# sunyzhi55/Diffusion_Models_Collection

Hardware: AMD Instinct MI355X
Metric: CIFAR-10 UNet DDPM train imgs/sec (aggregate over GPUs) (higher is better)
Workload: dtype bf16; 1 GPU; configs/cifar10_unet.py UNet DDPM train step at 32x32 (q_sample, fwd, MSE, bwd, clip, AdamW, EMA), dropout 0.1; model=UNet 37.06M (128ch, mult 1,2,2,2, attn 16/8), global_batch=128, per_gpu_batch=128, parallelism=dp1

## Files before the change

diffusion_models_collection_amd/_lib.py:

```python
import ctypes
import os
from pathlib import Path

import torch

_PKG = Path(__file__).resolve().parent
LIB_PATH = Path(os.environ.get("DMC_LIB", _PKG / "libdmc.so"))

DMC_F32, DMC_BF16 = 0, 1
MODE_NORMAL, MODE_UPSAMPLE, MODE_DILATE = 0, 1, 2
PRO_NONE, PRO_AFFINE_SILU, PRO_SILU, PRO_AFFINE, PRO_GN_SILU = 0, 1, 2, 3, 4
LOSS = {"l1": 0, "l2": 1, "huber": 2}
PRED = {"eps": 0, "v": 1}
OBJECTIVE_MAX_BLOCKS = 64
PACK_FWD, PACK_DGRAD, PACK_UPDGRAD = 0, 1, 2

_c_int, _c_p, _c_f, _c_u32, _c_long, _c_size = (ctypes.c_int, ctypes.c_void_p, ctypes.c_float, ctypes.c_uint32,
                                                ctypes.c_long, ctypes.c_size_t)


ACT_NONE, ACT_GELU, ACT_GELU_DROP, ACT_DGELU = 0, 1, 2, 3
FUSED_GN_STATS = 1


class ConvDesc(ctypes.Structure):
    _fields_ = [
        ("dtype", _c_int), ("N", _c_int), ("H", _c_int), ("W", _c_int),
        ("C1", _c_int), ("C2", _c_int), ("ld1", _c_int), ("ld2", _c_int), ("Kc", _c_int),
        ("OH", _c_int), ("OW", _c_int), ("Cout", _c_int), ("ntaps", _c_int), ("mode", _c_int), ("stride", _c_int),
        ("tap_dy", _c_int * 16), ("tap_dx", _c_int * 16),
        ("prologue", _c_int), ("pro_scale", _c_p), ("pro_shift", _c_p), ("ld_pro", _c_int),
        ("drop_seed", _c_u32), ("drop_thresh", _c_u32), ("drop_scale", _c_f), ("drop_ld", _c_int),
        ("drop_seed_base", _c_p),
        ("bias", _c_p), ("addvec", _c_p), ("ld_add", _c_int), ("resid", _c_p), ("ld_res", _c_int),
        ("silu_pre", _c_p), ("ld_silu", _c_int), ("Csplit", _c_int), ("ldy1", _c_int), ("ldy2", _c_int),
        ("out_f32", _c_int), ("out_nchw", _c_int), ("act", _c_int), ("y_pre", _c_p), ("ld_pre", _c_int),
        ("gn_part", _c_p), ("wg_bias", _c_p), ("pro_groups", _c_int), ("pro_eps", _c_f),
    ]


class WgradJob(ctypes.Structure):
    _fields_ = [("slab", ctypes.c_void_p), ("bslab", ctypes.c_void_p), ("dw", ctypes.c_void_p),
                ("dbias", ctypes.c_void_p), ("splits", ctypes.c_int), ("KK", ctypes.c_int), ("Cpad", ctypes.c_int),
                ("Cout", ctypes.c_int), ("Ctot", ctypes.c_int), ("ntaps", ctypes.c_int), ("Kc", ctypes.c_int),
                ("scale", ctypes.c_float), ("layout", ctypes.c_int)]
# ... 18 lines not shown
    _fields_ = [("w", _c_p), ("dst", _c_p), ("dtype", _c_int), ("mode", _c_int), ("Cout", _c_int), ("Cin", _c_int),
                ("kh", _c_int), ("kw", _c_int), ("Kc", _c_int), ("koff", _c_int)]


class TensorRef(ctypes.Structure):
    _fields_ = [("a", _c_p), ("b", _c_p), ("n", _c_long)]


def _load():
    if not LIB_PATH.exists():
        raise RuntimeError(
            f"libdmc.so not found at {LIB_PATH}. Build it with `python -m diffusion_models_collection_amd.build` "
            "(there is no fallback: the diffusion hot path runs only on the gfx950 HIP kernels).")
    lib = ctypes.CDLL(str(LIB_PATH))
    sig = {
        "dmc_version": (_c_int, []),
        "dmc_set_option": (_c_int, [ctypes.c_char_p, _c_long]),
        "dmc_get_option": (_c_long, [ctypes.c_char_p]),
        "dmc_reset_options": (None, [_c_int]),
        "dmc_last_error": (ctypes.c_char_p, []),
        "dmc_conv2d_workspace": (_c_size, [ctypes.POINTER(ConvDesc)]),
        "dmc_conv_halo_prologue": (_c_int, [ctypes.POINTER(ConvDesc)]),
        "dmc_conv2d_fused_epilogue": (_c_int, [ctypes.POINTER(ConvDesc), ctypes.c_size_t]),
        "dmc_conv2d": (_c_int, [ctypes.POINTER(ConvDesc), _c_p, _c_p, _c_p, _c_p, _c_p, _c_p, _c_size, _c_p]),
        "dmc_conv2d_wgrad_workspace": (_c_size, [ctypes.POINTER(ConvDesc)]),
        "dmc_conv2d_wgrad": (_c_int, [ctypes.POINTER(ConvDesc), _c_p, _c_int, _c_p, _c_p, _c_p, _c_p, _c_f, _c_p]),
        "dmc_conv2d_wgrad_partial": (_c_int, [ctypes.POINTER(ConvDesc), _c_p, _c_int, _c_p, _c_p, _c_p, _c_p, _c_f,
                                              ctypes.POINTER(WgradJob), _c_p]),
        "dmc_wgrad_reduce_batch": (_c_int, [ctypes.POINTER(WgradJob), _c_int, _c_p]),
        "dmc_conv2d_wgrad_group_ok": (_c_int, [ctypes.POINTER(ConvDesc), _c_int]),
        "dmc_conv2d_wgrad_group_workspace": (_c_size, [ctypes.POINTER(WgradGroupItem), _c_int,
                                                       ctypes.POINTER(_c_size)]),
        "dmc_conv2d_wgrad_group": (_c_int, [ctypes.POINTER(WgradGroupItem), _c_int, ctypes.POINTER(WgradJob), _c_p]),
        "dmc_wgrad_slab_bytes": (_c_long, [_c_int]),
        "dmc_pack_weight": (_c_int, [_c_int, _c_int, _c_p, _c_int, _c_int, _c_int, _c_int, _c_int, _c_p, _c_p]),
        "dmc_pack_tiles": (_c_int, [ctypes.POINTER(PackJob), _c_int, _c_p, _c_int]),
        "dmc_pack_weights": (_c_int, [_c_p, _c_p, _c_int, _c_p]),
        "dmc_gn_workspace": (_c_size, [_c_int, _c_int, _c_int, _c_int]),
        "dmc_gn_stats": (_c_int, [_c_int, _c_p, _c_p, _c_int, _c_int, _c_int, _c_int, _c_int, _c_int, _c_int, _c_f,
                                  _c_p, _c_p, _c_p, _c_p, _c_p, _c_p, _c_p]),
        "dmc_gn_finalize": (_c_int, [_c_p, _c_int, _c_p, _c_int, _c_int, _c_int, _c_int, _c_f, _c_p, _c_p, _c_p, _c_p,
                                     _c_p, _c_p]),
        "dmc_gn_stats_apply_ok": (_c_int, [_c_int, _c_int, _c_int, _c_int, _c_int, _c_int]),
        "dmc_gn_stats_apply": (_c_int, [_c_int, _c_p, _c_p, _c_int, _c_int, _c_int, _c_int, _c_int, _c_int, _c_int,
                                        _c_f, _c_p, _c_p, _c_p, _c_p, _c_p, _c_int, _c_u32, _c_p, _c_u32, _c_f, _c_p,
                                        _c_int, _c_p]),
# ... 143 lines not shown
```

diffusion_models_collection_amd/csrc/dmc_conv.hip:

```cpp
#include "dmc_conv_impl.h"

namespace {

template <typename T> DMC_DEV void load4(const char* p, size_t idx, float* v, bool f32);
template <typename T>
DMC_DEV void load4(const char* p, size_t idx, float* v, bool f32) {
  if (f32 || sizeof(T) == 4) {
    v4f x = *(const v4f*)(p + idx * 4);
    v[0] = x[0]; v[1] = x[1]; v[2] = x[2]; v[3] = x[3];
  } else {
    v2i x = *(const v2i*)(p + idx * 2);
    v[0] = bf2f((uint32_t)x[0] & 0xffffu); v[1] = bf2f((uint32_t)x[0] >> 16);
    v[2] = bf2f((uint32_t)x[1] & 0xffffu); v[3] = bf2f((uint32_t)x[1] >> 16);
  }
}
template <typename T>
DMC_DEV void store4(char* p, size_t idx, const float* v, bool f32) {
  if (f32 || sizeof(T) == 4) {
    v4f x = {v[0], v[1], v[2], v[3]};
    *(v4f*)(p + idx * 4) = x;
  } else {
    v2i x;
    x[0] = (int)f2bf2(v[0], v[1]);
    x[1] = (int)f2bf2(v[2], v[3]);
// ... 428 lines not shown
template <int AI, int BI, int BM>
DMC_DEV void glds_issue_buf(const ConvK& a, char* base, int c0, unsigned k2, int wave, const unsigned* o1,
                            const unsigned* o2, const unsigned* ob) {
  if (c0 < a.C1) {
    const __amdgpu_buffer_rsrc_t r = __builtin_amdgcn_make_buffer_rsrc((void*)a.x1, (short)0, a.x1_bytes, 0x00020000);
    const unsigned c2 = (unsigned)c0 * 2u;
#pragma unroll
    for (int j = 0; j < AI; ++j)
      __builtin_amdgcn_raw_ptr_buffer_load_lds(r, (LDS_AS void*)(base + (wave * AI + j) * 1024), 16, o1[j] + c2, 0, 0, 0);
  } else {
    const __amdgpu_buffer_rsrc_t r = __builtin_amdgcn_make_buffer_rsrc((void*)a.x2, (short)0, a.x2_bytes, 0x00020000);
    const unsigned c2 = (unsigned)(c0 - a.C1) * 2u;
#pragma unroll
    for (int j = 0; j < AI; ++j)
      __builtin_amdgcn_raw_ptr_buffer_load_lds(r, (LDS_AS void*)(base + (wave * AI + j) * 1024), 16, o2[j] + c2, 0, 0, 0);
  }
  const __amdgpu_buffer_rsrc_t rw = __builtin_amdgcn_make_buffer_rsrc((void*)a.w, (short)0, a.w_bytes, 0x00020000);
#pragma unroll
  for (int j = 0; j < BI; ++j)
    __builtin_amdgcn_raw_ptr_buffer_load_lds(rw, (LDS_AS void*)(base + BM * 128 + (wave * BI + j) * 1024), 16, ob[j] + k2, 0, 0, 0);
}

DMC_DEV void xcd_tile(int NB, int& mb, int& nb) {
  const int total = gridDim.x, bid = blockIdx.x, per = total >> 3;
  const int t = bid < (per << 3) ? (bid & 7) * per + (bid >> 3) : bid;
  mb = t / NB;
  nb = t - mb * NB;
}

__host__ __device__ inline bool reg_epi_ok(const ConvK& a) {
  return a.reg_epi && (a.gst || a.reg_epi >= 2) && a.dtype_bytes == 2 && !a.out_f32 && !a.out_nchw && !a.silu_pre && a.Csplit == a.Cout &&
         a.act == DMC_ACT_NONE && (a.Cout & 127) == 0 && (a.ldy1 & 7) == 0 &&
         (!a.resid || (a.ld_res & 7) == 0) && (a.M & 127) == 0 && (!a.gst || a.OHW % 64 == 0);
}
DMC_DEV void reg_epilogue(const ConvK& a, v4f (&acc)[4][4], int m0, int n0, int wm, int wn) {
  const int lane = threadIdx.x & 63, fr = lane & 15, fh = lane >> 4;
  const bool odd = fh & 1;
  v4i rra[4][2];
  v4f ba[4], eva[4];
  const int img0 = (m0 + wm * 64) / a.OHW;
#pragma unroll
  for (int i = 0; i < 4; ++i) {
    const int co = n0 + wn * 64 + i * 16 + fh * 4;
    const int cc = co - (odd ? 4 : 0);
#pragma unroll
    for (int jp = 0; jp < 2; ++jp) {
      rra[i][jp] = v4i{0, 0, 0, 0};
      if (a.resid) {
// ... 211 lines not shown
      reg_epilogue(a, acc, m0, n0, wm, wn);
      return;
    }
  }
  __syncthreads();
#pragma unroll
  for (int j = 0; j < 4; ++j)
#pragma unroll
    for (int i = 0; i < 4; ++i)
      *(v4f*)(lds + (wm * 64 + j * 16 + fr) * EP + (wn * 64 + i * 16 + fh * 4) * 4) = acc[i][j];
  __syncthreads();
  if (a.sk) {
    const int Cpad = gridDim.y * BN;
    float* slab = a.sk + (size_t)blockIdx.z * a.M * Cpad;
    for (int idx = threadIdx.x; idx < BM * BN / 4; idx += NW * 64) {
      const int pl = idx / (BN / 4), cg = idx - pl * (BN / 4);
      if (m0 + pl < a.M) *(v4f*)(slab + (size_t)(m0 + pl) * Cpad + n0 + cg * 4) = *(const v4f*)(lds + pl * EP + cg * 16);
    }
    return;
  }
  tile_epilogue<T, BM, BN, NW * 64>(a, lds, EP, m0, n0);
}

DMC_DEV void wait_vm_upto40(int n) {
  switch (n < 0 ? 0 : n) {
#define DMC_W(i) case i: __builtin_amdgcn_s_waitcnt(waitcnt_vm(i)); break;
    DMC_W(0) DMC_W(1) DMC_W(2) DMC_W(3) DMC_W(4) DMC_W(5) DMC_W(6) DMC_W(7) DMC_W(8) DMC_W(9) DMC_W(10)
    DMC_W(11) DMC_W(12) DMC_W(13) DMC_W(14) DMC_W(15) DMC_W(16) DMC_W(17) DMC_W(18) DMC_W(19) DMC_W(20)
    DMC_W(21) DMC_W(22) DMC_W(23) DMC_W(24) DMC_W(25) DMC_W(26) DMC_W(27) DMC_W(28) DMC_W(29) DMC_W(30)
    DMC_W(31) DMC_W(32) DMC_W(33) DMC_W(34) DMC_W(35) DMC_W(36) DMC_W(37) DMC_W(38) DMC_W(39)
#undef DMC_W
    default: __builtin_amdgcn_s_waitcnt(waitcnt_vm(40)); break;
  }
}

template <int NS>
__global__ __launch_bounds__(256, NS <= 2 ? 2 : 1) void gemm1x1_persist_kernel(ConvK a, int ntiles, int NB, int tpb) {
  using T = bf16_t;
  constexpr int BM = 128, BN = 128, AI = 4, BI = 4, SB = (BM + BN) * 128;
  __shared__ __attribute__((aligned(16))) char lds[NS * SB + 4096];
  float* const sbias = (float*)(lds + NS * SB);
  const int lane = threadIdx.x & 63;
  const int wave = __builtin_amdgcn_readfirstlane(threadIdx.x >> 6);
  const int wm = wave % 2, wn = wave / 2;
  const int lrow = lane >> 3, lc = (lane & 7) ^ lrow;
  const int fr = lane & 15, fh = lane >> 4;
  const int t_begin = blockIdx.x * tpb, t_end = min(ntiles, t_begin + tpb);
  if (t_begin >= t_end) return;
  const int kst = a.Kc / 64, total = (t_end - t_begin) * kst;
  for (int c = threadIdx.x; c < NB * BN; c += 256) sbias[c] = (a.bias && c < a.Cout) ? a.bias[c] : 0.f;
  __builtin_amdgcn_s_waitcnt(waitcnt_vm(0));

  unsigned o1[AI], o2[AI], ob[BI];
  int it_tile = -1;
  auto issue = [&](int S) {
    const int ti = t_begin + S / kst, k = S - (S / kst) * kst;
    if (ti != it_tile) {
      it_tile = ti;
      const int mb = ti / NB, nb = ti - mb * NB;
#pragma unroll
      for (int j = 0; j < AI; ++j) {
        const unsigned pix = (unsigned)(mb * BM + (wave * AI + j) * 8 + lrow);
        o1[j] = (pix * a.ld1 + lc * 8) * 2u;
        o2[j] = (pix * a.ld2 + lc * 8) * 2u;
      }
#pragma unroll
      for (int j = 0; j < BI; ++j) {
        const unsigned co = (unsigned)(nb * BN + (wave * BI + j) * 8 + lrow);
        ob[j] = (co * a.Kc + lc * 8) * 2u;
      }
    }
    glds_issue_buf<AI, BI, BM>(a, lds + (S % NS) * SB, k * 64, (unsigned)k * 128u, wave, o1, o2, ob);
  };
  int nvm = 0;
  int pos[NS];
#pragma unroll
  for (int q = 0; q < NS; ++q) pos[q] = 0;
  for (int q = 0; q < NS - 1 && q < total; ++q) {
    issue(q);
    nvm += AI + BI;
    pos[q] = nvm;
  }
  v4f acc[4][4];
#pragma unroll
  for (int i = 0; i < 4; ++i)
#pragma unroll
    for (int j = 0; j < 4; ++j) acc[i][j] = v4f{0.f, 0.f, 0.f, 0.f};
  for (int s = 0; s < total; ++s) {
    int mine = 0;
#pragma unroll
    for (int q = 0; q < NS; ++q)
      if (q == s % NS) mine = pos[q];
    wait_vm_upto40(nvm - mine);
    asm volatile("" ::: "memory");
    __builtin_amdgcn_sched_barrier(0);
    __builtin_amdgcn_s_barrier();
    __builtin_amdgcn_sched_barrier(0);
    asm volatile("" ::: "memory");
    v2i rres[4][4];
    const bool last = (s + 1) % kst == 0;
    if (a.resid && last) {
      const int t = t_begin + s / kst, mb = t / NB, nb = t - mb * NB;
#pragma unroll
      for (int i = 0; i < 4; ++i)
#pragma unroll
        for (int j = 0; j < 4; ++j) {
          const int co = nb * BN + wn * 64 + i * 16 + fh * 4, px = mb * BM + wm * 64 + j * 16 + fr;
          rres[i][j] = *(const v2i*)(a.resid + ((size_t)px * a.ld_res + co) * 2);
        }
      nvm += 16;
      asm volatile("" ::: "memory");
    }
    if (s + NS - 1 < total) {
      issue(s + NS - 1);
      nvm += AI + BI;
#pragma unroll
// ... 42 lines not shown
      for (int i = 0; i < 4; ++i) {
        const int co = n0 + wn * 64 + i * 16 + fh * 4;
        const v4f bv = *(const v4f*)(sbias + co);
#pragma unroll
        for (int j = 0; j < 4; ++j) {
          const int px = m0 + wm * 64 + j * 16 + fr;
          v4f v = acc[i][j] + bv;
          if (a.resid) {
            const v2i r = rres[i][j];
            v[0] += bf2f((uint32_t)r[0] & 0xffffu); v[1] += bf2f((uint32_t)r[0] >> 16);
            v[2] += bf2f((uint32_t)r[1] & 0xffffu); v[3] += bf2f((uint32_t)r[1] >> 16);
          }
          v2i o;
          o[0] = (int)f2bf2(v[0], v[1]);
          o[1] = (int)f2bf2(v[2], v[3]);
          *(v2i*)(ybase + ((size_t)px * ldy + co - cbase) * 2) = o;
          acc[i][j] = v4f{0.f, 0.f, 0.f, 0.f};
        }
      }
      nvm += 16;
      asm volatile("" ::: "memory");
      __builtin_amdgcn_sched_barrier(0);
    }
  }
}



template <int HP>
DMC_DEV void halo_issue(const ConvK& a, char* buf, int c0, int wave, int pb, int pe, const unsigned* h1,
                        const unsigned* h2) {
  const bool first = c0 < a.C1;
  const __amdgpu_buffer_rsrc_t r = __builtin_amdgcn_make_buffer_rsrc(
      first ? (void*)a.x1 : (void*)a.x2, (short)0, first ? a.x1_bytes : a.x2_bytes, 0x00020000);
  const unsigned c2 = (unsigned)(first ? c0 : c0 - a.C1) * 2u;
#pragma unroll
  for (int p = 0; p < HP; ++p)
    if (p >= pb && p < pe)
      __builtin_amdgcn_raw_ptr_buffer_load_lds(r, (LDS_AS void*)(buf + (wave * HP + p) * 1024), 16,
                                               (first ? h1[p] : h2[p]) + c2, 0, 0, 0);
}

DMC_DEV void halo_pro_load(const ConvK& a, int n, int c0, v4f* st) {
  const int lane = threadIdx.x & 63, lrow = lane >> 3, lc = (lane & 7) ^ lrow;
  const float* sc = a.psc + (size_t)n * a.ldp + c0 + lc * 8;
  const float* sh = a.psh + (size_t)n * a.ldp + c0 + lc * 8;
// ... 1153 lines not shown

bool epi_stats_ok(const ConvK& k, const void* ws, size_t ws_bytes) {
  if (k.dtype_bytes != 2 || k.out_f32 || k.out_nchw || k.silu_pre || k.Csplit != k.Cout || k.Cout % 128 ||
      k.M % 256 || k.OHW % 64 || ((k.Cout | k.ldy1 | k.ld_res) & 7))
    return false;
  if (!dmc::opt(dmc::OPT_NO_NARROW) && ((k.C2 == 0 && k.C1 <= 8 && k.Cout >= 16) || k.Cout <= 8)) {
    int R, nimg;
    return nin_plan(k, &R, &nimg) != 0;
  }
  if (dmc::opt(dmc::OPT_NO_GLDS) || dmc::opt(dmc::OPT_NO_EPI_STATS))
    return false;
  if (img_plan(k))
    return k.OH == 8 && k.act == DMC_ACT_NONE;
  if (k.prologue == DMC_PRO_AFFINE_SILU) {
    int R, nimg;
    return halo2_pro_plan(k, &R, &nimg) != 0;
  }
  if (k.prologue != DMC_PRO_NONE) return false;
  const FwdPlan p = plan_glds(k);
  return p.splits == 1 || ws == nullptr || ws_bytes < p.ws || dmc::opt(dmc::OPT_NO_SPLITK);
}


int gemm1x1_plan(const ConvK& k) {
  if (!dmc::opt(dmc::OPT_GEMM1X1) || k.dtype_bytes != 2 || k.ntaps != 1 || k.stride != 1 || k.mode != DMC_MODE_NORMAL ||
      k.tdy0 || k.tdx0 || k.H != k.OH || k.W != k.OW || k.prologue != DMC_PRO_NONE)
    return 0;
  if (k.C1 % 64 || k.C2 % 64 || k.Kc != k.C1 + k.C2 || k.x1_bytes == 0 || (k.C2 && k.x2_bytes == 0) || k.w_bytes == 0)
    return 0;
  if (k.addvec || (k.resid && (k.ld_res & 3)) || k.silu_pre || k.gst || k.gsk ||
      k.act != DMC_ACT_NONE || k.sk || k.out_f32 || k.out_nchw || (k.ldy1 & 3) || k.M % 128 ||
      k.Cout % 128 || k.Cout > 1024)
    return 0;
  if (k.Csplit != k.Cout && (k.Csplit % 128 || (k.ldy2 & 3) || !k.y2 || k.resid)) return 0;
  const long ntiles = (long)(k.M / 128) * (k.Cout / 128);
  if (ntiles < 128) return 0;
  const long blocks = 512;
  return (int)((ntiles + blocks - 1) / blocks);
}

template <typename T>
int launch_fwd(ConvK k, void* ws, size_t ws_bytes, hipStream_t s) {
  constexpr int EPC = TT<T>::KPL;
  DMC_REQUIRE(k.prologue != DMC_PRO_GN_SILU || img_plan(k),
              "conv: DMC_PRO_GN_SILU is taken only by the small-map conv (dmc_conv_halo_prologue says when)");
  if (!dmc::opt(dmc::OPT_NO_NARROW) && sizeof(T) == 2) {
    int R, nimg;
    if (k.C2 == 0 && k.C1 <= EPC && k.Cout >= 16 && nin_plan(k, &R, &nimg)) {
      if (reg_epi_ok(k)) conv3x3_nin_kernel<true><<<dim3(k.M / 128, k.Cout / 128), 256, 0, s>>>(k, R, nimg);
      else conv3x3_nin_kernel<false><<<dim3(k.M / 128, k.Cout / 128), 256, 0, s>>>(k, R, nimg);
      return dmc::check_launch("dmc_conv2d");
    }
    const int hp = k.Cout <= 8 ? nout_plan(k, &R, &nimg) : 0;
    if (hp) {
      const int npl = (k.C1 + k.C2) / 64;
      const dim3 g(k.M / 128);
      if (hp == 6) { if (npl == 1) conv3x3_nout_kernel<6, 1><<<g, 256, 0, s>>>(k, R, nimg); else conv3x3_nout_kernel<6, 2><<<g, 256, 0, s>>>(k, R, nimg); }
      else if (hp == 7) { if (npl == 1) conv3x3_nout_kernel<7, 1><<<g, 256, 0, s>>>(k, R, nimg); else conv3x3_nout_kernel<7, 2><<<g, 256, 0, s>>>(k, R, nimg); }
      else { if (npl == 1) conv3x3_nout_kernel<9, 1><<<g, 256, 0, s>>>(k, R, nimg); else conv3x3_nout_kernel<9, 2><<<g, 256, 0, s>>>(k, R, nimg); }
      return dmc::check_launch("dmc_conv2d");
    }
  }
  if (!dmc::opt(dmc::OPT_NO_NARROW)) {
    if (k.C2 == 0 && k.C1 <= EPC && k.Cout >= 16) {
      conv_narrow_in_kernel<T><<<dim3(dmc::cdiv(k.M, 256), dmc::cdiv(k.Cout, 32)), 256, 0, s>>>(k);
      return dmc::check_launch("dmc_conv2d");
    }
    if (k.Cout <= 8 && (k.C2 == 0 || k.C1 % EPC == 0)) {
      conv_narrow_out_kernel<T><<<dmc::cdiv(k.M, 256), 256, 0, s>>>(k);
      return dmc::check_launch("dmc_conv2d");
    }
  }
  if (sizeof(T) == 2) {
    const int bn = img_plan(k);
    if (bn) { launch_img(k, bn, s); return dmc::check_launch("dmc_conv2d"); }
  }
  if (sizeof(T) == 2) {
    const int tpb = gemm1x1_plan(k);
    if (tpb) {
      const int NB = k.Cout / 128, ntiles = (k.M / 128) * NB;
      gemm1x1_persist_kernel<2><<<dmc::cdiv(ntiles, tpb), 256, 0, s>>>(k, ntiles, NB, tpb);
      return dmc::check_launch("dmc_conv2d");
    }
  }
  if (sizeof(T) == 2 && k.prologue == DMC_PRO_AFFINE_SILU) {
    int R, nimg;
    const int hp2 = halo2_pro_plan(k, &R, &nimg);
    if (hp2) { launch_halo2<true>(k, hp2, R, nimg, s); return dmc::check_launch("dmc_conv2d"); }
  }
  if (sizeof(T) == 2 && k.prologue == DMC_PRO_NONE && !dmc::opt(dmc::OPT_NO_GLDS)) {
    FwdPlan p = plan_glds(k);
    if (p.splits > 1 && (ws == nullptr || ws_bytes < p.ws || dmc::opt(dmc::OPT_NO_SPLITK))) { p.splits = 1; p.cfg = 2; }
    if (p.splits > 1) { k.sk = (float*)ws; k.sk_per = p.per; }
    const bool buf = k.C1 % 64 == 0 && k.C2 % 64 == 0 && k.Kc == k.C1 + k.C2 && k.x1_bytes > 0 &&
                     (k.C2 == 0 || k.x2_bytes > 0) && k.w_bytes > 0 && !dmc::opt(dmc::OPT_NO_BUFLDS);
    int R2, nimg2;
    const int hp2 = (buf && p.splits == 1 && !dmc::opt(dmc::OPT_NO_HALO)) ? halo2_plan(k, &R2, &nimg2) : 0;
    if (hp2) launch_halo2<false>(k, hp2, R2, nimg2, s);
    else if (buf) launch_glds<true>(k, p, s);
    else launch_glds<false>(k, p, s);
    return dmc::check_launch("dmc_conv2d");
  }
  const RegPlan rp = plan_reg(k);
  if (rp.big) {
// ... 15 lines not shown
  return dmc::check_launch("dmc_conv2d");
}


}

extern "C" size_t dmc_conv2d_workspace(const dmc_conv_desc* d) {
  ConvK k;
  if (fill_convk(d, nullptr, nullptr, nullptr, nullptr, nullptr, k)) return 0;
  if (k.M == 0) return 0;
  if (d->dtype != DMC_BF16 || d->prologue != DMC_PRO_NONE || dmc::opt(dmc::OPT_NO_GLDS)) return plan_reg(k).ws;
  return plan_glds(k).ws;
}

extern "C" int dmc_conv2d_fused_epilogue(const dmc_conv_desc* d, size_t ws_bytes) {
  ConvK k;
  if (fill_convk(d, nullptr, nullptr, nullptr, nullptr, nullptr, k) || k.M == 0 || k.Cout == 0) return 0;
  const void* ws = ws_bytes ? (const void*)d : nullptr;
  int f = 0;
  if (k.OHW % 64 == 0 && k.Cout % 8 == 0 && epi_stats_ok(k, ws, ws_bytes)) f |= DMC_FUSED_GN_STATS;
  return f;
}

extern "C" int dmc_conv2d(const dmc_conv_desc* d, const void* x1, const void* x2, const void* w, void* y1,
                          void* y2, void* workspace, size_t ws_bytes, void* stream) {
  ConvK k;
  if (fill_convk(d, x1, x2, w, y1, y2, k)) return 1;
  hipStream_t s = dmc::as_stream(stream);
  if (k.M == 0 || k.Cout == 0) return 0;
  float* const part = d->gn_part;
  if (part) {
    DMC_REQUIRE(k.OHW % 64 == 0 && k.Cout % 8 == 0 && k.Csplit == k.Cout && !k.out_nchw && k.ldy1 % 4 == 0,
                "conv: GroupNorm partials need OH*OW %% 64 == 0, Cout %% 8 == 0 and one NHWC output");
    k.gst = epi_stats_ok(k, workspace, ws_bytes) ? part : nullptr;
  }
  int gsk_done = 0;
  if (part && !k.gst && !dmc::opt(dmc::OPT_NO_SKGN)) { k.gsk = part; k.gsk_done = &gsk_done; }
  const int rc = d->dtype == DMC_F32 ? launch_fwd<float>(k, workspace, ws_bytes, s)
                                     : launch_fwd<bf16_t>(k, workspace, ws_bytes, s);
  if (rc) return rc;
  if (!part || k.gst || gsk_done) return 0;
  const int nseg = k.M / 64, nch = k.Cout / 8;
  const int blocks = (int)(((long)nseg * nch + 3) / 4);
  if (k.out_f32 || d->dtype == DMC_F32)
    gn_part_kernel<float><<<blocks, 256, 0, s>>>(k.y1, k.ldy1, nseg, nch, part);
  else
// ... 53 lines not shown
```

diffusion_models_collection_amd/csrc/dmc_elem.hip:

```cpp
#include <stdlib.h>
#include <string.h>
#include "dmc_common.h"
#include "dmc_internal.h"

namespace dmc {
static thread_local char g_err[512] = "";
void set_error(const char* fmt, ...) {
  va_list ap;
  va_start(ap, fmt);
  vsnprintf(g_err, sizeof(g_err), fmt, ap);
  va_end(ap);
}
}

namespace dmc {
namespace {
struct OptDef {
  const char* name;
  long def;
};
constexpr OptDef kOpts[OPT_COUNT] = {
    {"DMC_NO_NARROW", 0}, {"DMC_NO_GLDS", 0}, {"DMC_NO_SPLITK", 0}, {"DMC_NO_BUFLDS", 0}, {"DMC_NO_HALO", 0},
    {"DMC_HALO_PRO", 1}, {"DMC_GN_STATS_SPLIT", 0}, {"DMC_GN_BWD_SPLIT", 0}, {"DMC_ATTN_STAGED", 0},
    {"DMC_ATTN_HG", 0}, {"DMC_WG_BLOCKS", 512}, {"DMC_GN_STATS_ONE_MAX", 1l << 20}, {"DMC_GN_BWD_ONE_MAX", 65536},
    {"DMC_NO_XCD", 0}, {"DMC_NO_EPI_STATS", 0}, {"DMC_WG_MINPIX", 0}, {"DMC_GN_BWD_SLICES", 2}, {"DMC_NO_SKGN", 0},
    {"DMC_WG_HALO_TARGET", 256}, {"DMC_SK_TARGET", 240}, {"DMC_SK_MAX", 8}, {"DMC_NO_NHALO", 0},
    {"DMC_GN_BWD_FUSED", 4}, {"DMC_GN_BWD_FUSED_MAXHW", 1l << 30}, {"DMC_GN_BWD_NT", 1024},
    {"DMC_REG_EPI", 3}, {"DMC_GEMM1X1", 1}, {"DMC_WG_PIPE", 1}, {"DMC_IMG_MASK", 15}, {"DMC_IMG_GN", 1}, {"DMC_WG_IMG4", 1},
};
struct OptTable {
  long v[OPT_COUNT];
  OptTable() { reset(true); }
  void reset(bool env) {
    for (int i = 0; i < OPT_COUNT; ++i) {
      v[i] = kOpts[i].def;
      const char* e = env ? getenv(kOpts[i].name) : nullptr;
      if (e && e[0]) v[i] = atol(e);
    }
  }
};
OptTable& table() {
  static OptTable t;
  return t;
}
}
long opt(Opt o) { return table().v[o]; }
}

extern "C" int dmc_set_option(const char* name, long value) {
  for (int i = 0; i < dmc::OPT_COUNT; ++i)
    if (strcmp(name, dmc::kOpts[i].name) == 0) {
// ... 897 lines not shown
```

diffusion_models_collection_amd/kernels.py:

```python
import ctypes

import torch

from . import _lib as L
from ._lib import LIB, check, ptr

TAPS3 = [(kh - 1, kw - 1) for kh in range(3) for kw in range(3)]
TAPS3_DGRAD = [(1 - kh, 1 - kw) for kh in range(3) for kw in range(3)]
TAPS1 = [(0, 0)]
TAPS_UPDGRAD = [(u - 1, v - 1) for u in range(4) for v in range(4)]


class Scratch:

    def __init__(self):
        self.bufs = {}

    def get(self, nbytes: int, device) -> torch.Tensor:
        nbytes = max(int(nbytes), 256)
        key = L.stream()
        buf = self.bufs.get(key)
        if buf is None or buf.numel() < nbytes:
            buf = torch.empty(int(nbytes * 1.25) + 4096, dtype=torch.uint8, device=device)
            self.bufs[key] = buf
# ... 84 lines not shown
        self.pending = []
        rows = sorted(agg.items(), key=lambda kv: -kv[1][1])
        tot = sum(v[1] for v in agg.values())
        lines = [f"conv launches: {tot / steps:.3f} ms/step"]
        for (kind, dt, N, H, W, Cin, OH, OW, Cout, nt, mode), (n, ms, fl) in rows:
            lines.append(f"{ms / steps * 1e3:8.1f} us/step  n/step {n / steps:4.1f}  avg {ms / n * 1e3:7.1f} us  "
                         f"{fl / (ms * 1e-3) / 1e12:7.1f} TF/s  {kind:5s} N{N} {H}x{W}x{Cin} -> {OH}x{OW}x{Cout} "
                         f"taps {nt} mode {mode}")
        return "\n".join(lines)


PROF = LayerProfile()


def conv(d, x1, x2, w, y1, y2=None):
    nbytes = LIB.dmc_conv2d_workspace(ctypes.byref(d))
    ws = SCRATCH.get(nbytes, y1.device) if nbytes else None
    PROF.wrap("conv", d, lambda: check(LIB.dmc_conv2d(ctypes.byref(d), ptr(x1), ptr(x2), ptr(w), ptr(y1), ptr(y2),
                                                      ptr(ws), nbytes, L.stream()), "dmc_conv2d"))


def conv_fused(d):
    return LIB.dmc_conv2d_fused_epilogue(ctypes.byref(d), LIB.dmc_conv2d_workspace(ctypes.byref(d)))


def upsample2x(dtype, x, C):
    N, H, W, ld = x.shape
    y = torch.empty(N, 2 * H, 2 * W, C, dtype=x.dtype, device=x.device)
    check(LIB.dmc_upsample2x_nhwc(L.dtype_code(dtype), ptr(x), N, H, W, C, ld, ptr(y), C, L.stream()),
          "dmc_upsample2x_nhwc")
    return y


def conv_halo_prologue(d):
    return bool(LIB.dmc_conv_halo_prologue(ctypes.byref(d)))


def _byte_span(t):
    n = 1 + sum((sz - 1) * st for sz, st in zip(t.shape, t.stride())) if t.numel() else 0
    return t.data_ptr(), t.data_ptr() + n * t.element_size()


class WgradDefer:

    def __init__(self):
        import os
# ... 720 lines not shown
```

include/dmc.h:

```cpp
#ifndef DMC_H
#define DMC_H
#include <stddef.h>
#include <stdint.h>
#ifdef __cplusplus
extern "C" {
#endif

enum { DMC_F32 = 0, DMC_BF16 = 1 };
enum { DMC_MODE_NORMAL = 0, DMC_MODE_UPSAMPLE = 1, DMC_MODE_DILATE = 2 };
enum { DMC_PRO_NONE = 0, DMC_PRO_AFFINE_SILU = 1, DMC_PRO_SILU = 2, DMC_PRO_AFFINE = 3, DMC_PRO_GN_SILU = 4 };
enum { DMC_LOSS_L1 = 0, DMC_LOSS_L2 = 1, DMC_LOSS_HUBER = 2 };
enum { DMC_PRED_EPS = 0, DMC_PRED_V = 1 };
#define DMC_OBJECTIVE_MAX_BLOCKS 64
enum { DMC_PACK_FWD = 0, DMC_PACK_DGRAD = 1, DMC_PACK_UPDGRAD = 2 };

int dmc_version(void);
const char* dmc_last_error(void);

int dmc_set_option(const char* name, long value);
long dmc_get_option(const char* name);
void dmc_reset_options(int from_env);

typedef struct dmc_conv_desc {
  int dtype;
// ... 17 lines not shown
  int ld_add;
  const void* resid;
  int ld_res;
  const float* silu_pre;
  int ld_silu;
  int Csplit;
  int ldy1, ldy2;
  int out_f32;
  int out_nchw;
  int act;
  void* y_pre;
  int ld_pre;
  float* gn_part;
  float* wg_bias;
  int pro_groups;
  float pro_eps;
} dmc_conv_desc;
enum { DMC_ACT_NONE = 0, DMC_ACT_GELU = 1, DMC_ACT_GELU_DROP = 2, DMC_ACT_DGELU = 3 };

size_t dmc_conv2d_workspace(const dmc_conv_desc* d);
int dmc_conv_halo_prologue(const dmc_conv_desc* d);
int dmc_conv2d_fused_epilogue(const dmc_conv_desc* d, size_t ws_bytes);
enum { DMC_FUSED_GN_STATS = 1 };
int dmc_conv2d(const dmc_conv_desc* d, const void* x1, const void* x2, const void* w,
               void* y1, void* y2, void* workspace, size_t ws_bytes, void* stream);

size_t dmc_conv2d_wgrad_workspace(const dmc_conv_desc* d);
int dmc_conv2d_wgrad(const dmc_conv_desc* d, const void* dy, int ld_dy, const void* x1,
                     const void* x2, void* workspace, float* dw, float scale, void* stream);
typedef struct dmc_wgrad_job {
  const float* slab;
  const float* bslab;
  float* dw;
  float* dbias;
  int splits, KK, Cpad, Cout, Ctot, ntaps, Kc;
  float scale;
  int layout;
} dmc_wgrad_job;
int dmc_conv2d_wgrad_partial(const dmc_conv_desc* d, const void* dy, int ld_dy, const void* x1, const void* x2,
                             void* workspace, float* dw, float scale, dmc_wgrad_job* job, void* stream);
int dmc_wgrad_reduce_batch(const dmc_wgrad_job* jobs, int njobs, void* stream);

#define DMC_WGRAD_GROUP_MAX 8
typedef struct dmc_wgrad_group_item {
  const dmc_conv_desc* d;
  const void* dy;
// ... 203 lines not shown
```

Before: 11860 img/s.

## Add panel-resident 1x1 GEMM kernel with weight ring for small-M convs

```diff
diff --git a/diffusion_models_collection_amd/_lib.py b/diffusion_models_collection_amd/_lib.py
--- a/diffusion_models_collection_amd/_lib.py
+++ b/diffusion_models_collection_amd/_lib.py
@@ -21,6 +21,7 @@
 
 ACT_NONE, ACT_GELU, ACT_GELU_DROP, ACT_DGELU = 0, 1, 2, 3
 FUSED_GN_STATS = 1
+GEMM1X1_TILE, GEMM1X1_RING, GEMM1X1_PANEL = 0, 1, 2
 
 
 class ConvDesc(ctypes.Structure):
@@ -85,6 +86,7 @@
         "dmc_conv2d_workspace": (_c_size, [ctypes.POINTER(ConvDesc)]),
         "dmc_conv_halo_prologue": (_c_int, [ctypes.POINTER(ConvDesc)]),
         "dmc_conv2d_fused_epilogue": (_c_int, [ctypes.POINTER(ConvDesc), ctypes.c_size_t]),
+        "dmc_conv2d_gemm1x1_form": (_c_int, [ctypes.POINTER(ConvDesc)]),
         "dmc_conv2d": (_c_int, [ctypes.POINTER(ConvDesc), _c_p, _c_p, _c_p, _c_p, _c_p, _c_p, _c_size, _c_p]),
         "dmc_conv2d_wgrad_workspace": (_c_size, [ctypes.POINTER(ConvDesc)]),
         "dmc_conv2d_wgrad": (_c_int, [ctypes.POINTER(ConvDesc), _c_p, _c_int, _c_p, _c_p, _c_p, _c_p, _c_f, _c_p]),
diff --git a/diffusion_models_collection_amd/csrc/dmc_conv.hip b/diffusion_models_collection_amd/csrc/dmc_conv.hip
--- a/diffusion_models_collection_amd/csrc/dmc_conv.hip
+++ b/diffusion_models_collection_amd/csrc/dmc_conv.hip
@@ -1,4 +1,5 @@
 #include "dmc_conv_impl.h"
+#include "dmc_gemm1x1_plan.h"
 
 namespace {
 
@@ -474,8 +475,7 @@
 }
 
 DMC_DEV void xcd_tile(int NB, int& mb, int& nb) {
-  const int total = gridDim.x, bid = blockIdx.x, per = total >> 3;
-  const int t = bid < (per << 3) ? (bid & 7) * per + (bid >> 3) : bid;
+  const int t = dmc_g1::xcd_order(blockIdx.x, gridDim.x);
   mb = t / NB;
   nb = t - mb * NB;
 }
@@ -733,15 +733,15 @@
   tile_epilogue<T, BM, BN, NW * 64>(a, lds, EP, m0, n0);
 }
 
-DMC_DEV void wait_vm_upto40(int n) {
+DMC_DEV void wait_vm_upto63(int n) {
   switch (n < 0 ? 0 : n) {
 #define DMC_W(i) case i: __builtin_amdgcn_s_waitcnt(waitcnt_vm(i)); break;
-    DMC_W(0) DMC_W(1) DMC_W(2) DMC_W(3) DMC_W(4) DMC_W(5) DMC_W(6) DMC_W(7) DMC_W(8) DMC_W(9) DMC_W(10)
-    DMC_W(11) DMC_W(12) DMC_W(13) DMC_W(14) DMC_W(15) DMC_W(16) DMC_W(17) DMC_W(18) DMC_W(19) DMC_W(20)
-    DMC_W(21) DMC_W(22) DMC_W(23) DMC_W(24) DMC_W(25) DMC_W(26) DMC_W(27) DMC_W(28) DMC_W(29) DMC_W(30)
-    DMC_W(31) DMC_W(32) DMC_W(33) DMC_W(34) DMC_W(35) DMC_W(36) DMC_W(37) DMC_W(38) DMC_W(39)
+#define DMC_W8(i) DMC_W(i) DMC_W(i + 1) DMC_W(i + 2) DMC_W(i + 3) DMC_W(i + 4) DMC_W(i + 5) DMC_W(i + 6) DMC_W(i + 7)
+    DMC_W8(0) DMC_W8(8) DMC_W8(16) DMC_W8(24) DMC_W8(32) DMC_W8(40) DMC_W8(48)
+    DMC_W(56) DMC_W(57) DMC_W(58) DMC_W(59) DMC_W(60) DMC_W(61) DMC_W(62)
+#undef DMC_W8
 #undef DMC_W
-    default: __builtin_amdgcn_s_waitcnt(waitcnt_vm(40)); break;
+    default: __builtin_amdgcn_s_waitcnt(waitcnt_vm(63)); break;
   }
 }
 
@@ -756,7 +756,7 @@
   const int wm = wave % 2, wn = wave / 2;
   const int lrow = lane >> 3, lc = (lane & 7) ^ lrow;
   const int fr = lane & 15, fh = lane >> 4;
-  const int t_begin = blockIdx.x * tpb, t_end = min(ntiles, t_begin + tpb);
+  const int t_begin = dmc_g1::xcd_order(blockIdx.x, gridDim.x) * tpb, t_end = min(ntiles, t_begin + tpb);
   if (t_begin >= t_end) return;
   const int kst = a.Kc / 64, total = (t_end - t_begin) * kst;
   for (int c = threadIdx.x; c < NB * BN; c += 256) sbias[c] = (a.bias && c < a.Cout) ? a.bias[c] : 0.f;
@@ -802,7 +802,7 @@
 #pragma unroll
     for (int q = 0; q < NS; ++q)
       if (q == s % NS) mine = pos[q];
-    wait_vm_upto40(nvm - mine);
+    wait_vm_upto63(nvm - mine);
     asm volatile("" ::: "memory");
     __builtin_amdgcn_sched_barrier(0);
     __builtin_amdgcn_s_barrier();
@@ -891,6 +891,187 @@
       asm volatile("" ::: "memory");
       __builtin_amdgcn_sched_barrier(0);
     }
+  }
+}
+
+template <int BM, int LDS>
+__global__ __launch_bounds__(256, 2) void gemm1x1_panel_kernel(ConvK a, int NB, int tps, int nsh, int nw) {
+  using T = bf16_t;
+  constexpr int J = BM / 32, AI = BM / 32, PB = BM * 128, WB = dmc_g1::kWSlice;
+  constexpr int NWMAX = dmc_g1::kWSlotsMax, PA = dmc_g1::kAhead;
+  __shared__ __attribute__((aligned(16))) char plds[LDS];
+  const int kst = a.Kc / 64;
+  char* const wring = plds + kst * PB;
+  float* const sbias = (float*)(wring + nw * WB);
+  const int lane = threadIdx.x & 63;
+  const int wave = __builtin_amdgcn_readfirstlane(threadIdx.x >> 6);
+  const int wm = wave % 2, wn = wave / 2;
+  const int lrow = lane >> 3, lc = (lane & 7) ^ lrow;
+  const int fr = lane & 15, fh = lane >> 4;
+  const int lb = dmc_g1::xcd_order(blockIdx.x, gridDim.x);
+  const int panel = lb / nsh, c_begin = (lb - panel * nsh) * tps, c_end = min(NB, c_begin + tps);
+  const int m0 = panel * BM;
+  const int total = (c_end - c_begin) * kst;
+
+  int nvm = 0;
+  {
+    const int nch = (c_end - c_begin) * 128, c = (wave * 64 + lane) * 4;
+    if (wave * 256 < nch) {
+      const unsigned off = (a.bias && c < nch) ? (unsigned)(c_begin * 128 + c) * 4u : kOOB;
+      dma_pieces<1>(a.bias ? (const void*)a.bias : (const void*)a.w, a.bias ? a.Cout * 4 : 0,
+                    (char*)sbias + wave * 1024, &off, 0u, 0, 1);
+      nvm += 1;
+    }
+  }
+
+  unsigned o1[AI], o2[AI], ob[4];
+#pragma unroll
+  for (int j = 0; j < AI; ++j) {
+    const unsigned pix = (unsigned)(m0 + (wave * AI + j) * 8 + lrow);
+    o1[j] = (pix * a.ld1 + lc * 8) * 2u;
+    o2[j] = (pix * a.ld2 + lc * 8) * 2u;
+  }
+  auto issue_a = [&](int k) {
+    const int c0 = k * 64;
+    char* const dst = plds + k * PB + wave * AI * 1024;
+    if (c0 < a.C1) dma_pieces<AI>(a.x1, a.x1_bytes, dst, o1, (unsigned)c0 * 2u, 0, AI);
+    else dma_pieces<AI>(a.x2, a.x2_bytes, dst, o2, (unsigned)(c0 - a.C1) * 2u, 0, AI);
+  };
+  int iw_c = c_begin, iw_k = 0, iw_slot = 0;
+  auto issue_w = [&]() {
+    if (iw_k == 0) {
+#pragma unroll
+      for (int j = 0; j < 4; ++j) {
+        const unsigned co = (unsigned)(iw_c * 128 + (wave * 4 + j) * 8 + lrow);
+        ob[j] = (co * a.Kc + lc * 8) * 2u;
+      }
+    }
+    dma_pieces<4>(a.w, a.w_bytes, wring + iw_slot * WB + wave * 4096, ob, (unsigned)iw_k * 128u, 0, 4);
+    if (++iw_k == kst) { iw_k = 0; ++iw_c; }
+    if (++iw_slot == nw) iw_slot = 0;
+  };
+  int posA[PA], posW[NWMAX];
+#pragma unroll
+  for (int q = 0; q < PA; ++q) posA[q] = 0;
+#pragma unroll
+  for (int q = 0; q < NWMAX; ++q) posW[q] = 0;
+  auto set_a = [&](int k) {
+#pragma unroll
+    for (int q = 0; q < PA; ++q)
+      if (q == (k & (PA - 1))) posA[q] = nvm;
+  };
+  auto set_w = [&](int slot) {
+#pragma unroll
+    for (int q = 0; q < NWMAX; ++q)
+      if (q == slot) posW[q] = nvm;
+  };
+  const int ahead = min(kst, PA);
+  for (int q = 0; q < ahead || (q < nw && q < total); ++q) {
+    if (q < ahead) { issue_a(q); nvm += AI; set_a(q); }
+    if (q < nw && q < total) { const int sl = iw_slot; issue_w(); nvm += 4; set_w(sl); }
+  }
+  v4f acc[4][J];
+#pragma unroll
+  for (int i = 0; i < 4; ++i)
+#pragma unroll
+    for (int j = 0; j < J; ++j) acc[i][j] = v4f{0.f, 0.f, 0.f, 0.f};
+  int k = 0, slot = 0, ct = c_begin;
+  for (int s = 0; s < total; ++s) {
+    int need = 0;
+#pragma unroll
+    for (int q = 0; q < NWMAX; ++q)
+      if (q == slot) need = posW[q];
+    if (s < kst) {
+#pragma unroll
+      for (int q = 0; q < PA; ++q)
+        if (q == (s & (PA - 1))) need = max(need, posA[q]);
+    }
+    wait_vm_upto63(nvm - need);
+    asm volatile("" ::: "memory");
+    __builtin_amdgcn_sched_barrier(0);
+    __builtin_amdgcn_s_barrier();
+    __builtin_amdgcn_sched_barrier(0);
+    asm volatile("" ::: "memory");
+    v2i rres[4][J];
+    const bool last = k + 1 == kst;
+    if (a.resid && last) {
+#pragma unroll
+      for (int i = 0; i < 4; ++i)
+#pragma unroll
+        for (int j = 0; j < J; ++j) {
+          const int co = ct * 128 + wn * 64 + i * 16 + fh * 4, px = m0 + wm * (BM / 2) + j * 16 + fr;
+          rres[i][j] = *(const v2i*)(a.resid + ((size_t)px * a.ld_res + co) * 2);
+        }
+      nvm += 4 * J;
+      asm volatile("" ::: "memory");
+    }
+    if (s + PA < kst) { issue_a(s + PA); nvm += AI; set_a(s + PA); }
+    if (s >= 1 && s + nw - 1 < total) { const int sl = iw_slot; issue_w(); nvm += 4; set_w(sl); }
+    const char* A = plds + k * PB;
+    const char* B = wring + slot * WB;
+    v4i fa[2][4], fb[2][J];
+#pragma unroll
+    for (int ks = 0; ks < 2; ++ks) {
+      const int chunk = ks * 4 + fh;
+#pragma unroll
+      for (int i = 0; i < 4; ++i) {
+        const int r = wn * 64 + i * 16 + fr;
+        fa[ks][i] = *(const v4i*)(B + r * 128 + ((chunk ^ (r & 7)) << 4));
+      }
+#pragma unroll
+      for (int j = 0; j < J; ++j) {
+        const int r = wm * (BM / 2) + j * 16 + fr;
+        fb[ks][j] = *(const v4i*)(A + r * 128 + ((chunk ^ (r & 7)) << 4));
+      }
+    }
+#pragma unroll
+    for (int ks = 0; ks < 2; ++ks)
+#pragma unroll
+      for (int i = 0; i < 4; ++i)
+#pragma unroll
+        for (int j = 0; j < J; ++j) acc[i][j] = mma16<T>(acc[i][j], fa[ks][i], fb[ks][j]);
+    __builtin_amdgcn_sched_group_barrier(0x100, 4 + J, 0);
+#pragma unroll
+    for (int g = 0; g < 4 + J; ++g) {
+      __builtin_amdgcn_sched_group_barrier(0x008, J / 2, 0);
+      __builtin_amdgcn_sched_group_barrier(0x100, 1, 0);
+    }
+    __builtin_amdgcn_sched_group_barrier(0x008, 8 * J - (4 + J) * (J / 2), 0);
+    if (last) {
+      asm volatile("" ::: "memory");
+      __builtin_amdgcn_sched_barrier(0);
+      const int n0 = ct * 128;
+      const bool second = n0 >= a.Csplit;
+      char* const ybase = second ? a.y2 : a.y1;
+      const int ldy = second ? a.ldy2 : a.ldy1, cbase = second ? a.Csplit : 0;
+#pragma unroll
+      for (int i = 0; i < 4; ++i) {
+        const int co = n0 + wn * 64 + i * 16 + fh * 4;
+        const v4f bv = *(const v4f*)(sbias + (co - c_begin * 128));
+#pragma unroll
+        for (int j = 0; j < J; ++j) {
+          const int px = m0 + wm * (BM / 2) + j * 16 + fr;
+          v4f v = acc[i][j] + bv;
+          if (a.resid) {
+            const v2i r = rres[i][j];
+            v[0] += bf2f((uint32_t)r[0] & 0xffffu); v[1] += bf2f((uint32_t)r[0] >> 16);
+            v[2] += bf2f((uint32_t)r[1] & 0xffffu); v[3] += bf2f((uint32_t)r[1] >> 16);
+          }
+          v2i o;
+          o[0] = (int)f2bf2(v[0], v[1]);
+          o[1] = (int)f2bf2(v[2], v[3]);
+          *(v2i*)(ybase + ((size_t)px * ldy + co - cbase) * 2) = o;
+          acc[i][j] = v4f{0.f, 0.f, 0.f, 0.f};
+        }
+      }
+      nvm += 4 * J;
+      asm volatile("" ::: "memory");
+      __builtin_amdgcn_sched_barrier(0);
+      k = 0; ++ct;
+    } else {
+      ++k;
+    }
+    if (++slot == nw) slot = 0;
   }
 }
 
@@ -2090,21 +2271,29 @@
 }
 
 
-int gemm1x1_plan(const ConvK& k) {
+dmc_g1::Plan gemm1x1_plan(const ConvK& k) {
+  dmc_g1::Plan none = {};
   if (!dmc::opt(dmc::OPT_GEMM1X1) || k.dtype_bytes != 2 || k.ntaps != 1 || k.stride != 1 || k.mode != DMC_MODE_NORMAL ||
       k.tdy0 || k.tdx0 || k.H != k.OH || k.W != k.OW || k.prologue != DMC_PRO_NONE)
-    return 0;
+    return none;
   if (k.C1 % 64 || k.C2 % 64 || k.Kc != k.C1 + k.C2 || k.x1_bytes == 0 || (k.C2 && k.x2_bytes == 0) || k.w_bytes == 0)
-    return 0;
+    return none;
   if (k.addvec || (k.resid && (k.ld_res & 3)) || k.silu_pre || k.gst || k.gsk ||
       k.act != DMC_ACT_NONE || k.sk || k.out_f32 || k.out_nchw || (k.ldy1 & 3) || k.M % 128 ||
       k.Cout % 128 || k.Cout > 1024)
-    return 0;
-  if (k.Csplit != k.Cout && (k.Csplit % 128 || (k.ldy2 & 3) || !k.y2 || k.resid)) return 0;
+    return none;
+  if (k.Csplit != k.Cout && (k.Csplit % 128 || (k.ldy2 & 3) || !k.y2 || k.resid)) return none;
   const long ntiles = (long)(k.M / 128) * (k.Cout / 128);
-  if (ntiles < 128) return 0;
-  const long blocks = 512;
-  return (int)((ntiles + blocks - 1) / blocks);
+  if (ntiles < 128) return none;
+  return dmc_g1::plan(k.M, k.Kc, k.Cout, (int)dmc::opt(dmc::OPT_GEMM1X1));
+}
+
+template <int BM>
+void launch_gemm1x1_panel(const ConvK& k, const dmc_g1::Plan& p, hipStream_t s) {
+  if (p.lds <= dmc_g1::kLdsLimit / 2)
+    gemm1x1_panel_kernel<BM, dmc_g1::kLdsLimit / 2><<<p.blocks, 256, 0, s>>>(k, k.Cout / 128, p.tps, p.nsh, p.nw);
+  else
+    gemm1x1_panel_kernel<BM, dmc_g1::kLdsLimit><<<p.blocks, 256, 0, s>>>(k, k.Cout / 128, p.tps, p.nsh, p.nw);
 }
 
 template <typename T>
@@ -2144,10 +2333,15 @@
     if (bn) { launch_img(k, bn, s); return dmc::check_launch("dmc_conv2d"); }
   }
   if (sizeof(T) == 2) {
-    const int tpb = gemm1x1_plan(k);
-    if (tpb) {
+    const dmc_g1::Plan gp = gemm1x1_plan(k);
+    if (gp.form == dmc_g1::FORM_PANEL) {
+      if (gp.BM == 128) launch_gemm1x1_panel<128>(k, gp, s);
+      else launch_gemm1x1_panel<64>(k, gp, s);
+      return dmc::check_launch("dmc_conv2d");
+    }
+    if (gp.form == dmc_g1::FORM_RING) {
       const int NB = k.Cout / 128, ntiles = (k.M / 128) * NB;
-      gemm1x1_persist_kernel<2><<<dmc::cdiv(ntiles, tpb), 256, 0, s>>>(k, ntiles, NB, tpb);
+      gemm1x1_persist_kernel<2><<<gp.blocks, 256, 0, s>>>(k, ntiles, NB, gp.tpb);
       return dmc::check_launch("dmc_conv2d");
     }
   }
@@ -2209,6 +2403,15 @@
   return f;
 }
 
+extern "C" int dmc_conv2d_gemm1x1_form(const dmc_conv_desc* d) {
+  ConvK k;
+  if (fill_convk(d, nullptr, nullptr, nullptr, nullptr, d->Csplit != d->Cout ? (void*)d : nullptr, k) || k.M == 0 ||
+      k.Cout == 0 || d->dtype != DMC_BF16 || d->gn_part)
+    return DMC_GEMM1X1_TILE;
+  if (img_plan(k)) return DMC_GEMM1X1_TILE;
+  return gemm1x1_plan(k).form;
+}
+
 extern "C" int dmc_conv2d(const dmc_conv_desc* d, const void* x1, const void* x2, const void* w, void* y1,
                           void* y2, void* workspace, size_t ws_bytes, void* stream) {
   ConvK k;
diff --git a/diffusion_models_collection_amd/csrc/dmc_elem.hip b/diffusion_models_collection_amd/csrc/dmc_elem.hip
--- a/diffusion_models_collection_amd/csrc/dmc_elem.hip
+++ b/diffusion_models_collection_amd/csrc/dmc_elem.hip
@@ -26,7 +26,7 @@
     {"DMC_NO_XCD", 0}, {"DMC_NO_EPI_STATS", 0}, {"DMC_WG_MINPIX", 0}, {"DMC_GN_BWD_SLICES", 2}, {"DMC_NO_SKGN", 0},
     {"DMC_WG_HALO_TARGET", 256}, {"DMC_SK_TARGET", 240}, {"DMC_SK_MAX", 8}, {"DMC_NO_NHALO", 0},
     {"DMC_GN_BWD_FUSED", 4}, {"DMC_GN_BWD_FUSED_MAXHW", 1l << 30}, {"DMC_GN_BWD_NT", 1024},
-    {"DMC_REG_EPI", 3}, {"DMC_GEMM1X1", 1}, {"DMC_WG_PIPE", 1}, {"DMC_IMG_MASK", 15}, {"DMC_IMG_GN", 1}, {"DMC_WG_IMG4", 1},
+    {"DMC_REG_EPI", 3}, {"DMC_GEMM1X1", 2}, {"DMC_WG_PIPE", 1}, {"DMC_IMG_MASK", 15}, {"DMC_IMG_GN", 1}, {"DMC_WG_IMG4", 1},
 };
 struct OptTable {
   long v[OPT_COUNT];
diff --git a/diffusion_models_collection_amd/csrc/dmc_gemm1x1_plan.h b/diffusion_models_collection_amd/csrc/dmc_gemm1x1_plan.h
--- /dev/null
+++ b/diffusion_models_collection_amd/csrc/dmc_gemm1x1_plan.h
@@ -0,0 +1,70 @@
+#pragma once
+
+#if defined(__HIPCC__)
+#define DMC_G1_HD __host__ __device__
+#else
+#define DMC_G1_HD
+#endif
+
+namespace dmc_g1 {
+
+enum { FORM_TILE = 0, FORM_RING = 1, FORM_PANEL = 2 };
+
+constexpr int kCus = 256;
+constexpr int kLdsLimit = 160 * 1024;
+constexpr int kWSlice = 128 * 128;
+constexpr int kWSlotsMin = 3, kWSlotsMax = 6;
+constexpr int kAhead = 8;
+
+DMC_G1_HD inline int xcd_order(int bid, int total) {
+  const int per = total >> 3;
+  return bid < (per << 3) ? (bid & 7) * per + (bid >> 3) : bid;
+}
+
+struct Plan {
+  int form;
+  int blocks;
+  int tpb;
+  int BM;
+  int nsh, tps;
+  int nw;
+  int lds;
+};
+
+inline int panel_lds(int BM, int K, int nw, int tps) {
+  return K / 64 * BM * 128 + nw * kWSlice + (tps * 128 * 4 + 1023) / 1024 * 1024;
+}
+
+inline Plan plan(long M, int K, int Cout, int want) {
+  Plan p = {};
+  const int NB = Cout / 128;
+  const long ntiles = M / 128 * NB;
+  p.form = FORM_RING;
+  p.tpb = (int)((ntiles + 511) / 512);
+  p.blocks = (int)((ntiles + p.tpb - 1) / p.tpb);
+  if (want < 2) return p;
+  int BM = 128;
+  if (panel_lds(128, K, kWSlotsMin, NB) > kLdsLimit || M / 128 < kCus) BM = 64;
+  if (panel_lds(BM, K, kWSlotsMin, NB) > kLdsLimit) return p;
+  const long panels = M / BM;
+  int nsh = panels >= kCus ? 1 : (int)((kCus + panels - 1) / panels);
+  if (nsh > NB) nsh = NB;
+  const int tps = (NB + nsh - 1) / nsh;
+  nsh = (NB + tps - 1) / tps;
+  const long blocks = panels * nsh;
+  if (want == 2 && !(M / 128 < kCus && tps == 1)) return p;
+  if (blocks > 0x7fffffffL / 2) return p;
+  int nw = tps * (K / 64) < kWSlotsMax ? tps * (K / 64) : kWSlotsMax;
+  if (nw < kWSlotsMin) nw = kWSlotsMin;
+  while (nw > kWSlotsMin && panel_lds(BM, K, nw, tps) > kLdsLimit) --nw;
+  if (blocks > kCus && panel_lds(BM, K, kWSlotsMin, tps) <= kLdsLimit / 2)
+    while (nw > kWSlotsMin && panel_lds(BM, K, nw, tps) > kLdsLimit / 2) --nw;
+  p.form = FORM_PANEL;
+  p.blocks = (int)blocks;
+  p.tpb = 0;
+  p.BM = BM; p.nsh = nsh; p.tps = tps; p.nw = nw;
+  p.lds = panel_lds(BM, K, nw, tps);
+  return p;
+}
+
+}
diff --git a/diffusion_models_collection_amd/kernels.py b/diffusion_models_collection_amd/kernels.py
--- a/diffusion_models_collection_amd/kernels.py
+++ b/diffusion_models_collection_amd/kernels.py
@@ -130,6 +130,10 @@
 
 def conv_fused(d):
     return LIB.dmc_conv2d_fused_epilogue(ctypes.byref(d), LIB.dmc_conv2d_workspace(ctypes.byref(d)))
+
+
+def conv_gemm1x1_form(d):
+    return LIB.dmc_conv2d_gemm1x1_form(ctypes.byref(d))
 
 
 def upsample2x(dtype, x, C):
diff --git a/include/dmc.h b/include/dmc.h
--- a/include/dmc.h
+++ b/include/dmc.h
@@ -63,6 +63,8 @@
 int dmc_conv_halo_prologue(const dmc_conv_desc* d);
 int dmc_conv2d_fused_epilogue(const dmc_conv_desc* d, size_t ws_bytes);
 enum { DMC_FUSED_GN_STATS = 1 };
+int dmc_conv2d_gemm1x1_form(const dmc_conv_desc* d);
+enum { DMC_GEMM1X1_TILE = 0, DMC_GEMM1X1_RING = 1, DMC_GEMM1X1_PANEL = 2 };
 int dmc_conv2d(const dmc_conv_desc* d, const void* x1, const void* x2, const void* w,
                void* y1, void* y2, void* workspace, size_t ws_bytes, void* stream);
 
```

Result: no change. 11860 img/s, median of 2 (-0.0%).
